# ruiqini/traj-opt-admm

Measured on AMD Instinct MI355X. Metric: ADMM iterations/sec, higher is better.
Workload: dtype f64

## Files before the change

### traj-opt-admm_amd/csrc/dev_common.h

```cpp
#pragma once
#include <hip/hip_runtime.h>
#include <stdint.h>
#include "dev_gjk.h"

namespace tj {

constexpr int WAVE = 64;
constexpr int STEP_CAP = 3332;
constexpr int NEWTON_CAP = 4000;
constexpr int MAX_LEVELS = 12;
constexpr int FRONT_CAP = 1024;

enum : int {
  ERR_PLANE_OVERFLOW = 1,
  ERR_FRONT_OVERFLOW = 2,
  ERR_LOOP_CAP = 4,
  ERR_PAIR_OVERFLOW = 8,
  ERR_NOT_SPD = 16,
  ERR_LS_RANGE = 32,
  ERR_CCD_STUCK = 128,
  ERR_SLACK_ARMIJO = 256,
  ERR_PLANE_REFINE = 64,
  ERR_PEER_TIMEOUT = 512,
  ERR_PASS_TIMEOUT = 1024,
// ... 85 lines not shown
  int rank[XCH_MAX];
  double* rx[XCH_MAX][2];
  unsigned long long* cnt[XCH_MAX];
};

struct Dev {
  int mode, U, P, res, S, T, N;
  int u0, u1;
  int rank, world;
  int xf;
  int c2_fold;
  int xf_all;
  __host__ __device__ int xf_want() const { return (xf_all || xs_async || fa_units) ? U : U - (u1 - u0); }
  __host__ __device__ int xf_units() const { return (xf && !xf_all) ? xf_want() * S : 0; }
  __host__ __device__ int xf_robot(int i) const { return xf_all ? i : (i < u0 ? i : i + (u1 - u0)); }
  int xch, xch_poll;
  const XchPeers* xp;
  int* xf_seg;
  double* rx[2];
  unsigned long long* xcnt;
  __host__ __device__ int n_foreign() const { return U - (u1 - u0); }
  __host__ __device__ int foreign_robot(int f) const { return f < u0 ? f : f + (u1 - u0); }
  __host__ __device__ int owner_of(int u) const { int r = (int)(((long long)(u + 1) * world - 1) / U); while ((long long)r * U / world > u) r--; while ((long long)(r + 1) * U / world <= u) r++; return r; }
  __host__ __device__ int owned_by(int r) const { return (int)((long long)(r + 1) * U / world) - (int)((long long)r * U / world); }
  int xs_async, xs_seq; int* xs_sync;
  __host__ __device__ int* xs_go() const { return xs_sync + ((size_t)2 * U + 1) * 32; }
  __host__ __device__ int* xs_ticket(int u) const { return xs_sync + (size_t)u * 32; }
  __host__ __device__ int* xs_flag(int u) const { return xs_sync + ((size_t)U + u) * 32; }
  __host__ __device__ int* xs_done() const { return xs_sync + (size_t)2 * U * 32; }
  __host__ __device__ static size_t xs_sync_ints(int U_) { return ((size_t)2 * U_ + 2) * 32; }
  int keep_async, keep_seq, keep_waves; int* keep_sync;
  __host__ __device__ int* keep_go() const { return keep_sync + 16 * 32; }
  __host__ __device__ static size_t keep_sync_ints() { return 17 * 32; }
  int fa, fa_units, fa_seq, fa_mid, fa_nls, fa_nfront; int* fa_sync;
  __host__ __device__ int* fa_res(int i) const { return fa_sync + (size_t)(i & 15) * 32; }
  __host__ __device__ int* fa_fdone(int i) const { return fa_sync + (size_t)(16 + (i & 15)) * 32; }
  __host__ __device__ int* fa_fstart(int i) const { return fa_sync + (size_t)(32 + (i & 15)) * 32; }
  __host__ __device__ int* fa_go(int i) const { return fa_sync + (size_t)(48 + (i & 63)) * 32; }
  __host__ __device__ int* fa_commit(int u) const { return fa_sync + (size_t)(112 + u) * 32; }
  __host__ __device__ int* fa_rec() const { return fa_sync + (size_t)(112 + U) * 32; }
  __host__ __device__ static size_t fa_sync_ints(int U_) { return (size_t)(113 + U_) * 32; }
  int lsc_follow;
  int xs_band;
  int seq_tree;
  int fuse;
  double lambda, margin, offset, mu, vel_limit, acc_limit, ks, kt, stop;
  int cap_obs, cap_self, cap_pairs;
  int optimal_plane;
  const double* basis;
  const double* convert;
  const double* mdyn;
  const double* kdop;
  const double* pow08;
  int prim;
  const double *px, *py, *pz;
  const double* tri;
  const float* leafbox;
  int nlevels;
  int bvh_skip;
  int lvl_off[MAX_LEVELS], lvl_n[MAX_LEVELS];
  const float* boxes;
  double *spline;
  double *p_slack;
  double *p_lambda;
  double *t_slack;
  double *t_lambda;
  double *piece_time;
  double *oplanes; int *ocount;
  double *splanes; int *scount;
  int *ocand, *ocand_n;
  double *ohull;
  int *obs_work, *obs_work_n;
  double *oraw; int *ostamp;
  double *hullinfo;
// ... 144 lines not shown
  sig_sent();
}
__device__ __forceinline__ void xf_wait_seg(const Dev& D, int kind, int tr) {
  const int want = D.xf_want();
  const int* w = xf_word(D, kind, tr);
  const long long lim = (D.xch || D.xs_async) ? WAIT_2S + WAIT_2S / 20 : WAIT_5MS + WAIT_SLACK * gridDim.x;
  if (!poll_until<2>([&] { return xf_load_i(w) >= want; }, lim)) wait_failed(D, ERR_LOOP_CAP | ERR_PASS_TIMEOUT);
}
template <int SLEEP = 2>
__device__ __forceinline__ void xs_wait(const Dev& D, const int* w, int want) {
  if (!poll_until<SLEEP>([&] { return xf_load_i(w) >= want; }, WAIT_2S)) wait_failed(D, ERR_LOOP_CAP | ERR_XS_TIMEOUT);
}
__device__ __forceinline__ int sum16(const int* base, int stride = 32) {
  int v = lane_id() < 16 ? xf_load_i(base + (size_t)lane_id() * stride) : 0;
  for (int o = 8; o > 0; o >>= 1) v += __shfl_xor(v, o);
  return __shfl(v, 0);
}
__device__ __forceinline__ void keep_wait(const Dev& D) {
  if (threadIdx.x < 64 && !poll_until<8>([&] { return sum16(D.keep_sync) >= D.keep_waves; }, WAIT_2S)) wait_failed(D, ERR_LOOP_CAP | ERR_XS_TIMEOUT);
  __syncthreads();
  asm volatile("" ::: "memory");
}
__device__ __forceinline__ void fa_wait16(const Dev& D, const int* base, int want) {
  if (!poll_until<4>([&] { return sum16(base) - want >= 0; }, WAIT_2S)) wait_failed(D, ERR_LOOP_CAP | ERR_XS_TIMEOUT);
}
__device__ __forceinline__ void fa_wait_flag(const Dev& D, const int* w, int want) {
  if (!poll_until<4>([&] { return xf_load_i(w) - want >= 0; }, WAIT_2S)) wait_failed(D, ERR_LOOP_CAP | ERR_XS_TIMEOUT);
}
__device__ __forceinline__ void fa_count(int* w) {
  sig_acked();
  if ((threadIdx.x & 63) == 0) __hip_atomic_fetch_add(w, 1, __ATOMIC_RELAXED, __HIP_MEMORY_SCOPE_AGENT);
  sig_sent();
}
__device__ __forceinline__ void xs_out(bool wt, double* p, double v) { if (wt) xf_store(p, v); else *p = v; }

constexpr int HULL_INFO_STRIDE = 128, HULL_BOX = 18, HULL_KLO = 24, HULL_KHI = 73;
__device__ __forceinline__ double* hull_record(const Dev& D, int u, int tr) { return D.hullinfo + ((size_t)u * D.S + tr) * HULL_INFO_STRIDE; }
__device__ __forceinline__ void hull_box_axis(const double* P, int a, double& lo, double& hi) {
  lo = INFINITY; hi = -INFINITY;
  for (int j = 0; j < 6; j++) { const double v = P[3 * j + a]; if (v < lo) lo = v; if (v > hi) hi = v; }
}
__device__ __forceinline__ void hull_kdop_axis(const Dev& D, const double* P, int ax, double& lo, double& up) {
  lo = INFINITY; up = -INFINITY;
  kdop_interval6(D.kdop[3 * ax], D.kdop[3 * ax + 1], D.kdop[3 * ax + 2], P, lo, up);
}
template <bool WT>
__device__ __forceinline__ void hull_record_put(const Dev& D, int u, int tr, int lane, double p, double blo, double bhi, double klo, double khi) {
  auto put = [](double* d, double v) { if constexpr (WT) xf_store(d, v); else *d = v; };
  double* o = hull_record(D, u, tr);
  if (lane < 18) put(o + lane, p);
  if (lane < 3) {
    put(o + HULL_BOX + lane, blo); put(o + HULL_BOX + 3 + lane, bhi);
    put(D.hbox + ((size_t)tr * 6 + lane) * D.U + u, blo); put(D.hbox + ((size_t)tr * 6 + 3 + lane) * D.U + u, bhi);
  }
  if (lane < 49) { put(o + HULL_KLO + lane, klo); put(o + HULL_KHI + lane, khi); }
}
template <bool WT>
__device__ __forceinline__ void hull_record_store(const Dev& D, int u, int tr, int lane, const double* P) {
  double blo = 0, bhi = 0, klo = 0, khi = 0;
  if (lane < 3) hull_box_axis(P, lane, blo, bhi);
  if (lane < 49) hull_kdop_axis(D, P, lane, klo, khi);
  hull_record_put<WT>(D, u, tr, lane, P[min(lane, 17)], blo, bhi, klo, khi);
}

__device__ __forceinline__ double* swept_record(const Dev& D, int u, int tr) { return D.ccdinfo + ((size_t)u * D.S + tr) * CCD_STRIDE; }
__device__ __forceinline__ BodySwept swept_body(const double* rec, double step) { return BodySwept{rec + CCD_P, rec + CCD_D, step}; }
// ... 81 lines not shown
```

### traj-opt-admm_amd/csrc/host_plan.h

```cpp
#pragma once
#include <algorithm>
#include <cstdlib>
#include <cstring>

namespace tj {

typedef const char* (*TuneFn)(const char* key);

struct KernelFact { int ok, regs, lds; };
struct PlanFacts {
  int num_cu;
  KernelFact xsolve;
  KernelFact grad[2];
  KernelFact front;
  int counters_on;
  int claim_refused;
  int prim, n_obs;
};
constexpr int PLAN_FACT_INTS = sizeof(PlanFacts) / sizeof(int);

struct HostPlan {
  size_t lds_grad = 0, lds_xs = 0, lds_xs2 = 0, lds_ls = 0, lds_seq = 0;
  LsLayout lsl;
  bool lsc_wide = false;
// ... 116 lines not shown
      auto gran = [](int r) { return (r + 7) / 8 * 8; };
      const int wx = XS_LOAD_THREADS / 64, wg = (h.grad_fold ? GRAD_FOLD_THREADS : GRAD_THREADS) / 64;
      const size_t lx = h.lds_xs + (size_t)ax.lds, lg = h.lds_grad_of(h.grad_fold, d.res) + (size_t)ag.lds;
      fits = ((wx + 3) / 4) * gran(ax.regs) + ((wg + 3) / 4) * gran(ag.regs) <= 512 && lx + lg <= (size_t)160 * 1024 && (wx + 3) / 4 + (wg + 3) / 4 <= 8;
    }
    if (!(2 * owned <= d.num_cu || (owned <= d.num_cu && fits))) d.xs_async = 0;
  }
  const char* const e_xs = tune("XS_ASYNC");
  const char* const e_keep = tune("KEEP_ASYNC");
  const bool xs_on = e_xs ? atoi(e_xs) != 0 : !f.counters_on, keep_on = e_keep ? atoi(e_keep) != 0 : !f.counters_on;
  d.xs_async = d.xs_async && xs_on;
  d.keep_async = (d.optimal_plane && decoupled && one && keep_on) ? 1 : 0;
  d.keep_waves = 1024;
  h.queues = 1 + d.xs_async + d.keep_async;
  h.forced = (e_xs && atoi(e_xs) != 0) || (e_keep && atoi(e_keep) != 0);
  if (f.claim_refused) { d.xs_async = 0; d.keep_async = 0; h.hwq_refused = true; }
  h.xs_two_queues = d.xs_async && tune("XS_ONE_QUEUE") == nullptr;
  h.keep_two_queues = d.keep_async != 0;
  if (const char* e = tune("GRAD_BALANCE")) d.grad_bal = (atoi(e) != 0 && owned * d.P <= 65536) ? 1 : 0;
  if (const char* e = tune("LS_HELP")) { h.ls_help_forced = true; h.ls_help_asked = atoi(e); }
  d.ls_help = plan_ls_help(d, h, d.num_cu);
  if (const char* e = tune("LS_HELP_LATE")) d.ls_help_late = std::max(0, std::min(4000, atoi(e)));
  d.ls_help_mute = flag(tune("LS_HELP_MUTE"), 0);
  d.fa = (d.xs_async && one && !d.optimal_plane &&
          (!coupled ? (d.fuse && owned * d.ls_help <= d.num_cu) : (h.lsc_wide && d.xf_all && owned * LSC_ROUNDS <= d.num_cu))) ? flag(tune("FRONT_ASYNC"), 1) : 0;
  h.fa_emulate = flag(tune("FRONT_ASYNC_ONE_QUEUE"), 0) != 0;
  if (d.fa) {
    h.fa_mid_front = plan_grids(d, h.n_solve_env).n_front;
    if (f.front.ok) {
      const int by_lds = (int)(((size_t)160 * 1024) / std::max<size_t>((size_t)f.front.lds, 1)), by_regs = 4 * (512 / std::max((f.front.regs + 7) / 8 * 8, 8)), per_cu = std::min(std::min(by_lds, by_regs), 32);
      h.fa_mid_ok = (long long)h.fa_mid_front <= (long long)(d.num_cu - 1) * per_cu;
    }
    h.fa_mid_ok = h.fa_mid_ok && flag(tune("FRONT_ASYNC_MID"), 1);
  }
  h.heal = flag(tune("HEAL"), 1) != 0;
  if (const char* e = tune("XS_FAULT")) h.xs_fault = atoi(e);
  if (h.lds_grad_of(true, d.res) > lds_max || h.lds_xs > lds_max || h.lds_ls > lds_max || h.lds_seq > lds_max)
    return fail("problem does not fit the 160 KB LDS of one CU (segments per robot / fleet size too large for this version)");
  return pl;
}

#ifdef TJ_KAT
inline int plan_record(const Plan& pl, const PlanFacts& f, int* out, int cap) {
  const Dev& d = pl.d; const HostPlan& h = pl.h;
  const Grids g = plan_grids(d, h.n_solve_env);
  const int v[] = {
    pl.err, d.mode, d.U, d.P, d.res, d.S, d.T, d.N, d.prim, d.u0, d.u1, d.rank, d.world, d.fuse, d.xf, d.xf_all, d.cap_obs, d.cap_self, d.cap_pairs, d.optimal_plane,
    d.pair_rows, d.cap_work, d.xs, d.grad_npl, d.xs_band, d.seq_tree, d.bvh_skip, d.pair_prio, d.mid_order, d.pair_lpw, d.pair_pass_on, d.spec, d.seq_fold, d.spec_budget,
    d.spec_min, d.ls_fast, d.num_cu, d.c2_fold, d.grad_bal, d.xs_async, d.keep_async, d.keep_waves, d.ls_help, d.ls_help_late, d.ls_help_mute, d.fa,
    h.grad_fold, h.n_solve_env, h.lsc_wide, h.fa_emulate, h.fa_mid_ok, h.fa_mid_front, h.hwq_refused, h.queues, h.forced, h.xs_two_queues, h.keep_two_queues, h.heal, h.xs_fault,
    (int)h.lds_grad, (int)h.lds_xs, (int)h.lds_xs2, (int)h.lds_ls, (int)h.lds_seq, (int)h.lsl.total, h.lsl.plane_cap, h.lsl.affine, h.lsl.groups,
    g.n_rows, g.n_ccd, g.n_xf, g.n_front, g.n_solve, g.n_obs_solve, g.n_mid_slack};
  const int nv = (int)(sizeof(v) / sizeof(int)), n = PLAN_FACT_INTS + nv;
  if (cap < n) return -n;
  memcpy(out, &f, sizeof(f)); memcpy(out + PLAN_FACT_INTS, v, sizeof(v));
  return n;
}
#endif

}
```

### traj-opt-admm_amd/csrc/kernels_pairs.h

```cpp
#pragma once
#include "dev_common.h"
#include "dev_linalg.h"
#include "kernels_sep.h"

namespace tj {

__global__ __launch_bounds__(64) void k_hullinfo(Dev D) {
  if (TJ_DONE(D)) return;
  const int u = blockIdx.x / D.S, tr = blockIdx.x % D.S, lane = lane_id();
  __shared__ double P[18];
  if (lane < 18) P[lane] = hull_entry(D, D.spline + (size_t)u * 3 * D.T, tr, lane / 3, lane % 3);
  __syncthreads();
  hull_record_store<false>(D, u, tr, lane, P);
}

__host__ __device__ inline int pair_units(int U, int R) {
  const int nc = (U + 63) / 64;
  int n = 0;
  for (int g = 0; 64 * g < U - 1; g++) { const int rows = min(64 * g + 64, U - 1) - 64 * g; n += ((rows + R - 1) / R) * (nc - g); }
  return n;
}
__host__ __device__ inline void pair_unit(int U, int R, int bid, int& tr, int& rb, int& cb) {
  const int per = pair_units(U, R), nc = (U + 63) / 64;
  tr = bid / per;
// ... 386 lines not shown
}
template <bool FA>
__device__ __forceinline__ void pair_dedicated(const Dev& D, int b, unsigned key, bool have_early, const PairSolve& early, bool head_start, int spec_thr, int epoch, int lane,
                                               double* A, double* B, const int* wpre) {
  auto ldi = [&](const int* p) { if constexpr (FA) return xf_load_i(p); else return *p; };
  __builtin_amdgcn_s_setprio(3);
  TJ_TIC(D, K_SEP_SELF_SOLVE, 0);
  const PairId id = pair_unkey(key);
  if (!pair_id_valid(D, id)) return;
  GjkState hs; bool hs_fin = false;
  if (!have_early) {
    pair_hull_put(A, B, lane, pair_hull_fetch<FA>(D, id, lane));
    spec_state_load<FA>(D, b, lane, hs, hs_fin);
  }
  const int cnt = wpre[id.tr + 1] - wpre[id.tr];
  const int* wl = D.pair_work + 3 * (size_t)id.tr * pair_work_cap_seg(D);
  bool member = false;
  for (int i = lane; i < cnt; i += 64) member = member || (ldi(wl + 3 * i + 1) == id.p0 && ldi(wl + 3 * i + 2) == id.q);
  __syncthreads();
  TJ_TIC(D, K_SEP_SELF_SOLVE, 1);
  PairSolve r = early;
  if (!have_early) r = pair_solve_wave(D, A, B, lane, hs, true, hs_fin);
#ifdef TJ_PHASE_TIMING
  if (lane == 0 && blockIdx.x < TJ_TIC_BLOCKS) { D.dbg[((size_t)K_SEP_SELF_SOLVE * TJ_TIC_BLOCKS + blockIdx.x) * TJ_TIC_SLOTS + 6] = r.gjk + 1000; D.dbg[((size_t)K_SEP_SELF_SOLVE * TJ_TIC_BLOCKS + blockIdx.x) * TJ_TIC_SLOTS + 7] = r.ok ? r.newton : -1; }
#endif
  if (ballot(member)) {
    if (lane == 0) atomicAdd(&D.ctl->spec_taken, 1);
    pair_note_slow(D, id, r.gjk, epoch, lane, head_start, spec_thr);
    pair_result_store(D, id, r, epoch, lane);
  }
  TJ_TIC(D, K_SEP_SELF_SOLVE, 2);
}
template <bool FA>
__device__ __forceinline__ void pair_generic(const Dev& D, int r, int Wg, int n, const SpecTags& tags, bool head_start, int spec_thr, int epoch, int lane,
                                             double* A, double* B, const int* wpre) {
  auto ldi = [&](const int* p) { if constexpr (FA) return xf_load_i(p); else return *p; };
  if (r >= n) return;
  TJ_TIC(D, K_SEP_SELF_SOLVE, 0);
  int it_tr = 0, it_p0 = 0, it_q = 0;
  const int n_mine = (n - r + Wg - 1) / Wg;
  if (n_mine > 64) { if (lane == 0) atomicOr(&D.ctl->error, ERR_PAIR_OVERFLOW); return; }
  if (lane < n_mine) {
    const size_t sl = (size_t)pair_work_slot(D, wpre, r + lane * Wg);
    it_tr = ldi(D.pair_work + 3 * sl); it_p0 = ldi(D.pair_work + 3 * sl + 1); it_q = ldi(D.pair_work + 3 * sl + 2);
  }
  auto item = [&](int j) { return PairId{__builtin_amdgcn_readlane(it_tr, j), __builtin_amdgcn_readlane(it_p0, j), __builtin_amdgcn_readlane(it_q, j)}; };
  PairId next = item(0);
  double hv = pair_hull_fetch<FA>(D, next, lane);
  for (int j = 0; j < n_mine; j++) {
    const bool first = j == 0;
    __syncthreads();
    pair_hull_put(A, B, lane, hv);
    __syncthreads();
    const PairId id = next;
    if (j + 1 < n_mine) {
      next = item(j + 1);
      hv = pair_hull_fetch<FA>(D, next, lane);
    }
    if (first) TJ_TIC(D, K_SEP_SELF_SOLVE, 1);
    if (head_start && tags.holds(pair_tag_word(epoch, pair_key(id)))) continue;
    GjkState gs;
    const PairSolve s = pair_solve_wave(D, A, B, lane, gs, false, false,
#ifdef TJ_PHASE_LIGHT
                                        nullptr);
#else
                                        first ? &D : nullptr);
#endif
#ifdef TJ_PHASE_TIMING
    if (lane == 0 && first && blockIdx.x < TJ_TIC_BLOCKS) { D.dbg[((size_t)K_SEP_SELF_SOLVE * TJ_TIC_BLOCKS + blockIdx.x) * TJ_TIC_SLOTS + 6] = s.gjk; D.dbg[((size_t)K_SEP_SELF_SOLVE * TJ_TIC_BLOCKS + blockIdx.x) * TJ_TIC_SLOTS + 7] = s.ok ? s.newton : -1; }
#endif
    pair_note_slow(D, id, s.gjk, epoch, lane, head_start, spec_thr);
    pair_result_store(D, id, s, epoch, lane);
    if (first) TJ_TIC(D, K_SEP_SELF_SOLVE, 2);
  }
}

template <bool FA = false>
__device__ __forceinline__ void sep_self_solve_body(const Dev& D, int bid, int nwaves, bool head_start, double* tile) {
  const int lane = lane_id();
  __shared__ double A[18], B[18];
  __shared__ int wpre[513];
  auto ldt = [&](const unsigned long long* p) { if constexpr (FA) return __hip_atomic_load(p, __ATOMIC_RELAXED, __HIP_MEMORY_SCOPE_AGENT); else return *p; };
  const int n_ded = min(nwaves / 2, SPEC_CAP);
  bool have_early = false; PairSolve early{false, false, 0, 0, 0, 0, 0, 0};
  if constexpr (FA) {
    if (head_start && bid < n_ded) have_early = pair_early_head_start(D, bid, lane, A, B, early);
    fa_wait_flag(D, D.fa_go(bid), D.fa_seq);
  }
  const unsigned long long spec_tag0 = head_start ? ldt(D.spec_tag + lane) : 0ull, spec_tag1 = head_start ? ldt(D.spec_tag + 64 + lane) : 0ull;
  const int spec_thr = head_start ? max(D.spec_min, D.ctl->gjk_prev - SPEC_GJK_WINDOW) : 0;
  const int n = pair_work_prefix<FA>(D, wpre, lane);
  const int epoch = D.ctl->epoch;
  if (n > 4 * nwaves) {
    const PairLanePlan pl = pair_lane_plan(D, n, nwaves);
    if (pl.pass_on && bid >= pl.np) pair_consumer<FA>(D, bid - pl.np, pl, nwaves, epoch, lane, A, B);
    else pair_lane_producer<FA>(D, bid, nwaves, n, pl, epoch, lane, wpre, tile);
    return;
  }
  const SpecTags tags = spec_tags(spec_tag0, spec_tag1, head_start, epoch, n_ded, lane);
  if (tags.dedicated(bid)) pair_dedicated<FA>(D, bid, tags.key_of(bid), have_early, early, head_start, spec_thr, epoch, lane, A, B, wpre);
  else pair_generic<FA>(D, bid - tags.below(bid), nwaves - tags.count(), n, tags, head_start, spec_thr, epoch, lane, A, B, wpre);
}
__global__ __launch_bounds__(64) void k_sep_self_solve(Dev D) {
  if (TJ_DONE(D)) return;
  __shared__ double tile[PAIR_TILE_DOUBLES];
  sep_self_solve_body(D, blockIdx.x, gridDim.x, false, tile);
}

__device__ __forceinline__ void compact_segment(const Dev& D, int u, int tr, int lane, double* pst_o = nullptr, double* pst_s = nullptr, int* cnt = nullptr, int pst_cap = 0, int* fits = nullptr) {
  const int U = D.U, epoch = D.ctl->epoch;
  const size_t seg = (size_t)u * D.S + tr;
  const bool obs_part = !(D.optimal_plane && !D.multi());
  const bool pair_part = D.multi();
  const int n = obs_part ? D.ocand_n[seg] : 0;
  const int W = (U + 63) >> 6;
  unsigned long long* bw = D.pairbits + ((size_t)tr * U + u) * W;
  unsigned long long wbits = 0;
  if (pair_part && lane < W) wbits = bw[lane];
  double* outp = D.splanes + seg * D.cap_self * 4;
  int pbase = 0;
  if (pair_part) {
    for (int q0 = 0; q0 < U; q0 += 64) {
      const unsigned long long word = __shfl(wbits, q0 >> 6);
      if (word == 0ull) continue;
      const int q = q0 + lane;
      const bool bit = (word >> lane) & 1ull;
      const size_t slot = ((size_t)tr * U + u) * U + min(q, U - 1);
      int st = 0; double v0 = 0, v1 = 0, v2 = 0, v3 = 0;
      if (bit && q < U) { st = D.pairstamp[slot]; const double* p = D.pairplane + 4 * slot; v0 = p[0]; v1 = p[1]; v2 = p[2]; v3 = p[3]; }
      const bool ok = bit && q < U && q != u && st == epoch;
      const unsigned long long mask = ballot(ok);
      const int idx = pbase + prefix_count(mask);
      if (ok) {
        if (idx < D.cap_self) {
// ... 44 lines not shown
```

### traj-opt-admm_amd/csrc/kernels_step.h

```cpp
#pragma once
#include "dev_common.h"
#include "dev_linalg.h"
#include "kernels_sep.h"
#include "kernels_ls.h"
#include "kernels_pairs.h"
#include "dev_dyntree.h"

namespace tj {

template <bool XF = false>
__device__ __forceinline__ void ccd_prep_segment(const Dev& D, const double* net, const double* dir, int u, int tr, int lane, double* sh, int sysdir = 0) {
  double* P = sh; double* Dh = sh + 18; double* PD = sh + 36; double* PS = sh + 54;
  auto ldd = [&](const double* p) { return (XF && sysdir == 1) ? xch_load(p) : ((XF && sysdir == 2) ? xf_load(p) : *p); };
  auto st = [&](double* p, double v) { if constexpr (XF) xf_store(p, v); else *p = v; };
  const int e = lane % 18, r0 = div_small(tr, D.res) * 3 + D.T * (e % 3);
  const double* B = D.basis + (size_t)tr * 36 + (e / 3) * 6;
  if (lane < 18) P[lane] = hull_sum(B, net + r0);
  else if (lane < 54) {
    double dk[6];
#pragma unroll
    for (int k = 0; k < 6; k++) dk[k] = ldd(dir + r0 + k);
    if (lane < 36) Dh[e] = hull_sum(B, dk); else PD[e] = hull_sum_pd(B, net + r0, dk);
  }
  blk_sync<true>();
// ... 549 lines not shown
  __host__ __device__ __forceinline__ int total() const { return obs + pt.count(); }
  __host__ __device__ __forceinline__ explicit FrontLayout(const Dev& d) : pt(d) {
    ord = d.grad_bal ? ((d.u1 - d.u0) * d.P + 63) / 64 : 0;
    xf = ord + d.xf_units();
    spec = xf + (d.spec ? SPEC_CAP : 0);
    obs = spec + owned_segments(d);
  }
};
struct MidLayout {
  enum Body { SLACK, PAIR, OBS };
  __host__ __device__ __forceinline__ static int slack_blocks(const Dev& d) { return (d.u1 - d.u0) * d.P; }
  int watcher, slack0, n_slack, pair0, n_pair, obs0, n_obs, total;
  __host__ __device__ __forceinline__ MidLayout(const Dev& d, int n_pair_waves, int n_obs_waves, bool with_watcher, bool slack_last) {
    watcher = with_watcher ? 1 : 0; n_slack = slack_blocks(d); n_pair = n_pair_waves; n_obs = n_obs_waves;
    pair0 = slack_last ? 0 : n_slack; obs0 = pair0 + n_pair; slack0 = slack_last ? obs0 + n_obs : 0;
    total = watcher + n_slack + n_pair + n_obs;
  }
  __host__ __device__ __forceinline__ Body body(int b) const { return (unsigned)(b - slack0) < (unsigned)n_slack ? SLACK : ((unsigned)(b - pair0) < (unsigned)n_pair ? PAIR : OBS); }
};
struct CcdLayout {
  int fin, xf, obs; PairTiles pt;
  __host__ __device__ __forceinline__ explicit CcdLayout(const Dev& d) : pt(d) {
    fin = d.seq_fold ? 1 : 0;
    xf = fin + d.xf_units();
    obs = xf + owned_segments(d);
  }
  __host__ __device__ __forceinline__ int tiles() const { return pt.count(); }
  __host__ __device__ __forceinline__ int total() const { return obs + tiles(); }
};
template <int PRIM, bool FA = false>
__global__ __launch_bounds__(64) void k_front(Dev D) {
  if (D.keep_seq > 0 && blockIdx.x == 0 && threadIdx.x == 0) __hip_atomic_store(D.keep_go(), D.keep_seq, __ATOMIC_RELAXED, __HIP_MEMORY_SCOPE_AGENT);
  int fa_epoch = 0;
  if constexpr (FA) {
    if (threadIdx.x == 0) __hip_atomic_fetch_add(D.fa_fstart(blockIdx.x), 1, __ATOMIC_RELAXED, __HIP_MEMORY_SCOPE_AGENT);
    fa_epoch = xf_load_i(D.fa_rec() + 1);
    if (xf_load_i(D.fa_rec() + 2) | (D.ctl->error & ERR_XS_TIMEOUT)) { fa_count(D.fa_fdone(blockIdx.x)); return; }
  } else if (TJ_DONE(D)) return;
  TJ_TIC(D, K_FRONT, 0);
  __shared__ double lds[OBS_LDS_DOUBLES > PAIR_LDS_DOUBLES ? OBS_LDS_DOUBLES : PAIR_LDS_DOUBLES];
  static_assert(sizeof(lds) >= GRAD_ORDER_CHUNK * sizeof(int), "grad_order_body stages its costs in this buffer");
  const FrontLayout L(D);
  const int bx = (int)blockIdx.x;
  const bool pub = D.xf_all != 0 || (D.fa_units != 0 && D.multi());
  if (bx < L.ord) grad_order_body<FA>(D, bx, (int*)lds);
  else if (bx < L.xf) xf_hull_body(D, bx - L.ord);
  else if (bx < L.spec) spec_pair_body<FA>(D, bx - L.xf, lds, fa_epoch);
  else if (bx < L.obs) obs_query_body<PRIM, FA>(D, bx - L.spec, lds, !pub, pub);
  else sep_self_rows_body<FA>(D, bx - L.obs, lds, D.xf != 0 || D.fa_units != 0);
  TJ_TIC(D, K_FRONT, 1);
  if constexpr (FA) fa_count(D.fa_fdone(blockIdx.x));
}
__global__ __launch_bounds__(64) void k_fa_gate(Dev D, int want) { fa_wait16(D, D.fa_res(0), want); }
template <int PRIM, bool FA, bool SLACK_LAST>
__device__ __forceinline__ void mid_dispatch(const Dev& D, int b, int n_pair_waves, int n_obs_waves, double* mid_lds) {
  const MidLayout L(D, n_pair_waves, n_obs_waves, FA, SLACK_LAST);
  const MidLayout::Body body = L.body(b);
  if (body == MidLayout::SLACK) { if (D.ctl->slack_now) slack_body(D, b - L.slack0, 1, mid_lds); TJ_TIC(D, K_MID, 1); return; }
  if (TJ_DONE(D)) return;
  if (body == MidLayout::PAIR) sep_self_solve_body<FA>(D, b - L.pair0, n_pair_waves, D.spec != 0, mid_lds);
  else { if constexpr (FA) { fa_wait_flag(D, D.fa_go(b), D.fa_seq); if constexpr (!SLACK_LAST) TJ_TIC(D, K_MID, 4); } obs_solve_body<PRIM, FA>(D, b - L.obs0, n_obs_waves); }
  TJ_TIC(D, K_MID, 1);
}
template <int PRIM, bool FA = false>
__global__ __launch_bounds__(64) __attribute__((amdgpu_waves_per_eu(2, 2))) void k_mid(Dev D, int n_pair_waves, int n_obs_waves) {
  constexpr int watcher = FA ? 1 : 0;
  if constexpr (FA) {
    if ((int)blockIdx.x < watcher) {
      fa_wait16(D, D.fa_fdone(0), (int)((unsigned)D.fa_seq * (unsigned)D.fa_nfront));
      sig_acked();
      xf_store_i(D.fa_go(threadIdx.x), D.fa_seq);
      sig_sent();
      return;
    }
  }
  const int b = (int)blockIdx.x - watcher;
  TJ_TIC(D, K_MID, 0);
#ifdef TJ_PHASE_TIMING
  if (threadIdx.x == 0 && blockIdx.x < TJ_TIC_BLOCKS) {
    D.dbg[((size_t)K_MID * TJ_TIC_BLOCKS + blockIdx.x) * TJ_TIC_SLOTS + 2] = __builtin_amdgcn_s_getreg((31 << 11) | 4);
    D.dbg[((size_t)K_MID * TJ_TIC_BLOCKS + blockIdx.x) * TJ_TIC_SLOTS + 3] = __builtin_amdgcn_s_getreg((31 << 11) | 20);
  }
#endif
  __shared__ double mid_lds[SLACK_LDS_DOUBLES > PAIR_TILE_DOUBLES ? SLACK_LDS_DOUBLES : PAIR_TILE_DOUBLES];
// ... 92 lines not shown
```

### traj-opt-admm_amd/csrc/tj_api.hip

```cpp
#include <hip/hip_runtime.h>
#include <cstdio>
#include <cstdlib>
#include <cstring>
#include <strings.h>
#include <string>
#include <type_traits>
#include <vector>
#include "../../include/trajadmm.h"
#include "dev_common.h"
#include "host_tables.h"
#include "kernels_sep.h"
#include "kernels_pairs.h"
#include "kernels_keep.h"
#include "kernels_newton.h"
#include "kernels_step.h"
#ifdef TJ_KAT
#include "../../include/trajadmm_kat.h"
#include "kernels_debug.h"
#endif
#include "kernels_plan.h"
#include "kernels_bvh.h"
#include "kernels_audit.h"
#include "kernels_audit_timed.h"
#include "kernels_closest.h"
// ... 202 lines not shown
  return TJ_OK;
}


int ensure_hull_cache(tj_ctx* c);

int flush_deferred(tj_ctx* c) {
  if (!c->maybe_deferred) return TJ_OK;
  const Dev& d = c->d;
  TJ_LAUNCH(k_flush, dim3(1), dim3(1), 0, c->stream, d, c->begin_folded ? 1 : 0);
  c->begin_folded = false;
  TJ_LAUNCH(k_slack, dim3((d.u1 - d.u0) * d.P), dim3(64), 0, c->stream, d, 1);
  HIPCHK(c, hipGetLastError());
  c->maybe_deferred = false;
  return TJ_OK;
}

#define QUIESCE_NOHEAL(c)                                       \
  do {                                                          \
    int qr_ = flush_deferred(c);                                \
    if (qr_) return qr_;                                        \
    HIPCHK(c, hipStreamSynchronize((c)->stream));               \
    if ((c)->xq.stream2) HIPCHK(c, hipStreamSynchronize((c)->xq.stream2)); \
    if ((c)->xq.stream3) HIPCHK(c, hipStreamSynchronize((c)->xq.stream3)); \
  } while (0)
#define QUIESCE(c)                                              \
  do {                                                          \
    QUIESCE_NOHEAL(c);                                          \
    if ((c)->snap_iters > 0 && !(c)->heal_busy) { int hr_ = heal_check(c, -1); if (hr_) return hr_; } \
  } while (0)

int restart_pairings(tj_ctx* c, bool keep_go) {
  HIPCHK(c, hipMemsetAsync(c->d.xs_sync, 0, (keep_go ? (size_t)(c->d.xs_go() - c->d.xs_sync) : Dev::xs_sync_ints(c->d.U)) * sizeof(int), c->stream));
  HIPCHK(c, hipMemsetAsync(c->d.fa_sync, 0, Dev::fa_sync_ints(c->d.U) * sizeof(int), c->stream)); c->ss.fa_seq = 0; c->ss.fa_armed = c->ss.fa_mid_now = false;
  if (!keep_go) { HIPCHK(c, hipMemsetAsync(c->d.keep_sync, 0, Dev::keep_sync_ints() * sizeof(int), c->stream)); c->ss.xs_seq = c->ss.xs_seq_gated = c->ss.keep_seq = 0; }
  return TJ_OK;
}
int checkpoint_take(tj_ctx* c, bool in_begin) {
  Checkpoint& k = c->ck;
  c->ss.ck_in_begin = in_begin; k.begin_folded = c->begin_folded; k.maybe_deferred = c->maybe_deferred; k.lsc_base = c->ss.lsc_base;
  if (!in_begin) { hipLaunchKernelGGL(k_snapshot, dim3(64, std::max(k.n, 1)), dim3(256), 0, c->stream, k.tab, k.n, 0, c->d.ctl, k.ctl); HIPCHK(c, hipGetLastError()); }
  return TJ_OK;
}
int checkpoint_restore(tj_ctx* c) {
  const Checkpoint& k = c->ck;
  hipLaunchKernelGGL(k_snapshot, dim3(64, std::max(k.n, 1)), dim3(256), 0, c->stream, k.tab, k.n, 1, c->d.ctl, k.ctl); HIPCHK(c, hipGetLastError());
  c->begin_folded = k.begin_folded; c->maybe_deferred = k.maybe_deferred; c->ss.lsc_base = k.lsc_base; c->hull_valid = c->ss.ccd_valid = c->ss.xf_used[0] = c->ss.xf_used[1] = false;
  return c->begin_folded ? flush_deferred(c) : TJ_OK;
}
void checkpoint_drop(tj_ctx* c) { c->ss.ck_in_begin = 0; }

int heal_check(tj_ctx* c, int err_known) {
  int err = err_known;
  if (err < 0) HIPCHK(c, hipMemcpy(&err, &c->d.ctl->error, sizeof(int), hipMemcpyDeviceToHost));
  const long long n = c->snap_iters; c->snap_iters = 0;
  if (!(err & ERR_XS_TIMEOUT)) { checkpoint_drop(c); return TJ_OK; }
  struct Busy { tj_ctx* c; ~Busy() { c->heal_busy = false; } } busy{c}; c->heal_busy = true;
  c->async_fallbacks++;
  release_queues(c);
  c->ss.xs_two_queues = c->ss.keep_two_queues = false; c->ss.xs_fault = 0;
  int r = restart_pairings(c, false);
  if (r || (r = checkpoint_restore(c))) return r;
  checkpoint_drop(c);
  HIPCHK(c, hipMemsetAsync(c->d.xf_seg, 0, (size_t)2 * c->d.S * XF_SEG_STRIDE * sizeof(int), c->stream)); HIPCHK(c, hipMemsetAsync(c->d.spec_n, 0, 8, c->stream));
  if ((r = tj_iterate_async(c, (int)n))) return r;
  QUIESCE_NOHEAL(c);
  return TJ_OK;
// ... 157 lines not shown
    if (!r) r = upload(c, q, src, n * sizeof(*q));
    dst = q;
    return r;
  };
  int r;
  if ((r = put(d.basis, t.basis.data(), t.basis.size())) || (r = put(d.convert, t.convert.data(), t.convert.size())) || (r = put(d.mdyn, t.mdyn, 36)) ||
      (r = put(d.kdop, t.kdop, 147)) || (r = put(d.pow08, t.pow08.data(), t.pow08.size())) || (r = put(d.xs_gather, gt.data(), gt.size()))) return r;
  return TJ_OK;
}

struct ArrayDecl { void** slot; size_t n, elem; bool snap; };
template <class T>
ArrayDecl arr(T*& p, size_t n, bool snap = false) { return ArrayDecl{(void**)&p, n, sizeof(T), snap}; }
constexpr bool SNAP = true;

std::vector<ArrayDecl> device_arrays(Dev& d) {
  const size_t U = d.U, S = d.S, P = d.P, T = d.T, owned = d.u1 - d.u0, n = 9 * P - 2, co = d.cap_obs, cs = d.cap_self;
  const bool multi = d.mode >= 1;
  std::vector<ArrayDecl> a = {
    arr(d.spline, U * 3 * T, SNAP), arr(d.p_slack, U * 18 * P, SNAP), arr(d.p_lambda, U * 18 * P, SNAP), arr(d.t_slack, U * P, SNAP), arr(d.t_lambda, U * P, SNAP), arr(d.piece_time, U, SNAP),
    arr(d.oplanes, U * S * co * 4), arr(d.ocount, U * S), arr(d.splanes, U * S * cs * 4), arr(d.scount, U * S),
    arr(d.lg, U * P * 19), arr(d.lh, U * P * 361), arr(d.xdir, U * d.xs, SNAP),
    arr(d.k_obs, U), arr(d.k_self, U), arr(d.step_out, U, SNAP), arr(d.ls_hist, U, SNAP), arr(d.grad_cost, owned * P), arr(d.grad_perm, owned * P), arr(d.ls_tab, U * LS_TAB_STRIDE), arr(d.ls_word, U),
    arr(d.ccdinfo, U * S * CCD_STRIDE), arr(d.pair_list, ACT_CAP),
    arr(d.seg_stats, U * S * 6, SNAP), arr(d.pair_stats, U * S * 2, SNAP), arr(d.blk_stats, U * P + U, SNAP),
    arr(d.hullinfo, U * S * HULL_INFO_STRIDE), arr(d.hbox, S * 6 * U), arr(d.cbox, S * 6 * U), arr(d.pairplane, multi ? S * U * U * 4 : 1),
    arr(d.pairstamp, multi ? S * U * U : 1), arr(d.pairbits, multi ? S * U * ((U + 63) / 64) : 1),
    arr(d.pair_work, 3 * (size_t)d.cap_work), arr(d.pair_work_n, S + 1), arr(d.pair_ovf, 4), arr(d.seq_gmem_d, SeqLayout(d.U, ACT_CAP, true).tree_doubles), arr(d.seq_gmem_i, SeqLayout(d.U, ACT_CAP, true).tree_ints),
    arr(d.spec_n, 2), arr(d.spec_list, 2 * SPEC_CAP), arr(d.spec_tag, SPEC_CAP), arr(d.spec_state, SPEC_CAP * SPEC_STATE_DOUBLES), arr(d.spec_sti, SPEC_CAP * SPEC_STATE_INTS),
    arr(d.pair_ovf_list, (size_t)d.cap_work + PAIR_CONSUMERS_MAX), arr(d.ctl, 1),
    arr(d.ocand, U * S * co), arr(d.ocand_n, U * S), arr(d.ohull, U * S * 18),
    arr(d.obs_work, 2 * U * S * co), arr(d.obs_work_n, 1), arr(d.oraw, U * S * co * 4), arr(d.ostamp, U * S * co),
    arr(d.grad_scr, owned * P * 16 * (co + cs)), arr(d.xs_scr, d.xs_band ? owned * (n * n + 4 * n) : 1),
    arr(d.xf_seg, 2 * S * XF_SEG_STRIDE), arr(d.xs_sync, Dev::xs_sync_ints(d.U)), arr(d.keep_sync, Dev::keep_sync_ints()), arr(d.fa_sync, Dev::fa_sync_ints(d.U))};
#ifdef TJ_PHASE_TIMING
  a.push_back(arr(d.dbg, (size_t)K_COUNT * TJ_TIC_BLOCKS * TJ_TIC_SLOTS));
#endif
  if (d.optimal_plane) {
    const bool m0 = d.mode == 0;
    a.insert(a.end(), {arr(d.kobs_id, m0 ? U * S * co : 1, m0), arr(d.kobs_n, U * S, m0), arr(d.kobs_cd, m0 ? U * S * co * 4 : 1, m0),
                       arr(d.kpair_on, m0 ? 1 : S * U * U, !m0), arr(d.kpair_list, m0 ? 1 : S * U * U, !m0), arr(d.kpair_n, 2, !m0), arr(d.kpair_cd, m0 ? 1 : S * U * U * 4, !m0)});
  }
  if (d.mode == TJ_MODE_MULTI_COUPLED)
    a.insert(a.end(), {arr(d.xL, U * (d.xs_band ? (n - 1) * BAND_BS + n : n * n)), arr(d.xy, U * n), arr(d.xg, U * n), arr(d.xcorner, U * 4), arr(d.k_obs_f, U), arr(d.ls_e, (size_t)LSC_ROUNDS * U * LS_GROUPS)});
  return a;
}

int allocate_arrays(tj_ctx* c) {
  const std::vector<ArrayDecl> arrays = device_arrays(c->d);
  int r;
  for (const ArrayDecl& a : arrays) if ((r = dalloc_bytes(c, a.slot, std::max<size_t>(a.n, 1) * a.elem))) return r;
  std::vector<SnapRegion> tab;
  for (const ArrayDecl& a : arrays) {
    if (!a.snap) continue;
    char* snap = nullptr;
    if ((r = dalloc(c, &snap, (a.n * a.elem + 15) / 16 * 16))) return r;
    tab.push_back(SnapRegion{(char*)*a.slot, snap, (unsigned long long)(a.n * a.elem)});
  }
  c->ck.n = (int)tab.size();
  if ((r = dalloc(c, &c->ck.tab, tab.size())) || (r = dalloc(c, &c->ck.ctl, 1)) || (r = upload(c, c->ck.tab, tab.data(), tab.size() * sizeof(SnapRegion)))) return r;
  return TJ_OK;
}

}

extern "C" {

// ... 1628 lines not shown
```

Baseline: 6185.

## Release pair-solve waves per segment as front tiles finish

```diff
diff --git a/traj-opt-admm_amd/csrc/dev_common.h b/traj-opt-admm_amd/csrc/dev_common.h
--- a/traj-opt-admm_amd/csrc/dev_common.h
+++ b/traj-opt-admm_amd/csrc/dev_common.h
@@ -141,14 +141,17 @@
   int keep_async, keep_seq, keep_waves; int* keep_sync;
   __host__ __device__ int* keep_go() const { return keep_sync + 16 * 32; }
   __host__ __device__ static size_t keep_sync_ints() { return 17 * 32; }
-  int fa, fa_units, fa_seq, fa_mid, fa_nls, fa_nfront; int* fa_sync;
+  int fa, fa_units, fa_seq, fa_mid, fa_nls, fa_nfront, pair_seg, fa_ntile; int* fa_sync;
   __host__ __device__ int* fa_res(int i) const { return fa_sync + (size_t)(i & 15) * 32; }
   __host__ __device__ int* fa_fdone(int i) const { return fa_sync + (size_t)(16 + (i & 15)) * 32; }
   __host__ __device__ int* fa_fstart(int i) const { return fa_sync + (size_t)(32 + (i & 15)) * 32; }
   __host__ __device__ int* fa_go(int i) const { return fa_sync + (size_t)(48 + (i & 63)) * 32; }
   __host__ __device__ int* fa_commit(int u) const { return fa_sync + (size_t)(112 + u) * 32; }
   __host__ __device__ int* fa_rec() const { return fa_sync + (size_t)(112 + U) * 32; }
-  __host__ __device__ static size_t fa_sync_ints(int U_) { return (size_t)(113 + U_) * 32; }
+  __host__ __device__ int* fa_seg(int tr) const { return fa_sync + (size_t)(113 + U + tr) * 32; }
+  __host__ __device__ int* fa_hs() const { return fa_sync + (size_t)(113 + U + S) * 32; }
+  __host__ __device__ int* fa_listed(int par) const { return fa_sync + (size_t)(114 + U + S) * 32 + (size_t)par * (((size_t)S + 32) & ~(size_t)31); }
+  __host__ __device__ static size_t fa_sync_ints(int U_, int S_) { return (size_t)(114 + U_ + S_) * 32 + 2 * (((size_t)S_ + 32) & ~(size_t)31); }
   int lsc_follow;
   int xs_band;
   int seq_tree;
@@ -359,6 +362,14 @@
   if ((threadIdx.x & 63) == 0) __hip_atomic_fetch_add(w, 1, __ATOMIC_RELAXED, __HIP_MEMORY_SCOPE_AGENT);
   sig_sent();
 }
+__device__ __forceinline__ void fa_count2(int* group, int* w) {
+  sig_acked();
+  if ((threadIdx.x & 63) == 0) {
+    if (group) __hip_atomic_fetch_add(group, 1, __ATOMIC_RELAXED, __HIP_MEMORY_SCOPE_AGENT);
+    __hip_atomic_fetch_add(w, 1, __ATOMIC_RELAXED, __HIP_MEMORY_SCOPE_AGENT);
+  }
+  sig_sent();
+}
 __device__ __forceinline__ void xs_out(bool wt, double* p, double v) { if (wt) xf_store(p, v); else *p = v; }
 
 constexpr int HULL_INFO_STRIDE = 128, HULL_BOX = 18, HULL_KLO = 24, HULL_KHI = 73;
diff --git a/traj-opt-admm_amd/csrc/host_plan.h b/traj-opt-admm_amd/csrc/host_plan.h
--- a/traj-opt-admm_amd/csrc/host_plan.h
+++ b/traj-opt-admm_amd/csrc/host_plan.h
@@ -172,6 +172,8 @@
       h.fa_mid_ok = (long long)h.fa_mid_front <= (long long)(d.num_cu - 1) * per_cu;
     }
     h.fa_mid_ok = h.fa_mid_ok && flag(tune("FRONT_ASYNC_MID"), 1);
+    d.fa_ntile = d.mode >= 1 ? pair_units(d.U, d.pair_rows) : 0;
+    d.pair_seg = (h.fa_mid_ok && d.mode >= 1 && d.fa_ntile > 0) ? flag(tune("PAIR_SEG_RELEASE"), 1) : 0;
   }
   h.heal = flag(tune("HEAL"), 1) != 0;
   if (const char* e = tune("XS_FAULT")) h.xs_fault = atoi(e);
diff --git a/traj-opt-admm_amd/csrc/kernels_pairs.h b/traj-opt-admm_amd/csrc/kernels_pairs.h
--- a/traj-opt-admm_amd/csrc/kernels_pairs.h
+++ b/traj-opt-admm_amd/csrc/kernels_pairs.h
@@ -442,32 +442,25 @@
   TJ_TIC(D, K_SEP_SELF_SOLVE, 2);
 }
 template <bool FA>
-__device__ __forceinline__ void pair_generic(const Dev& D, int r, int Wg, int n, const SpecTags& tags, bool head_start, int spec_thr, int epoch, int lane,
-                                             double* A, double* B, const int* wpre) {
-  auto ldi = [&](const int* p) { if constexpr (FA) return xf_load_i(p); else return *p; };
-  if (r >= n) return;
-  TJ_TIC(D, K_SEP_SELF_SOLVE, 0);
-  int it_tr = 0, it_p0 = 0, it_q = 0;
-  const int n_mine = (n - r + Wg - 1) / Wg;
-  if (n_mine > 64) { if (lane == 0) atomicOr(&D.ctl->error, ERR_PAIR_OVERFLOW); return; }
-  if (lane < n_mine) {
-    const size_t sl = (size_t)pair_work_slot(D, wpre, r + lane * Wg);
-    it_tr = ldi(D.pair_work + 3 * sl); it_p0 = ldi(D.pair_work + 3 * sl + 1); it_q = ldi(D.pair_work + 3 * sl + 2);
-  }
+__device__ __forceinline__ void pair_solve_items(const Dev& D, int n_mine, int it_tr, int it_p0, int it_q, const SpecTags& tags, bool head_start, int spec_thr, int epoch, int lane,
+                                                 double* A, double* B, bool stamps) {
+  if (n_mine <= 0) return;
   auto item = [&](int j) { return PairId{__builtin_amdgcn_readlane(it_tr, j), __builtin_amdgcn_readlane(it_p0, j), __builtin_amdgcn_readlane(it_q, j)}; };
+  auto listed = [&](const PairId& id) { return (unsigned)id.tr < (unsigned)D.S && (unsigned)id.p0 < (unsigned)D.U && (unsigned)id.q < (unsigned)D.U; };
   PairId next = item(0);
-  double hv = pair_hull_fetch<FA>(D, next, lane);
+  double hv = listed(next) ? pair_hull_fetch<FA>(D, next, lane) : 0.0;
   for (int j = 0; j < n_mine; j++) {
-    const bool first = j == 0;
+    const bool first = stamps && j == 0;
     __syncthreads();
     pair_hull_put(A, B, lane, hv);
     __syncthreads();
     const PairId id = next;
     if (j + 1 < n_mine) {
       next = item(j + 1);
-      hv = pair_hull_fetch<FA>(D, next, lane);
+      hv = listed(next) ? pair_hull_fetch<FA>(D, next, lane) : 0.0;
     }
     if (first) TJ_TIC(D, K_SEP_SELF_SOLVE, 1);
+    if (!listed(id)) continue;
     if (head_start && tags.holds(pair_tag_word(epoch, pair_key(id)))) continue;
     GjkState gs;
     const PairSolve s = pair_solve_wave(D, A, B, lane, gs, false, false,
@@ -484,6 +477,94 @@
     if (first) TJ_TIC(D, K_SEP_SELF_SOLVE, 2);
   }
 }
+__device__ __forceinline__ int pair_prefix_row(const int* pre, int S, int x) {
+  int lo = 0, hi = S;
+  while (hi - lo > 1) { const int mid = (lo + hi) >> 1; if (pre[mid] <= x) lo = mid; else hi = mid; }
+  return lo;
+}
+template <class F>
+__device__ __forceinline__ void pair_prefix_of(int S, int* pre, int lane, F&& f) {
+  int run = 0;
+  for (int base = 0; base < S; base += 64) {
+    const int tr = base + lane;
+    const int c = tr < S ? f(tr) : 0;
+    int x = c;
+#pragma unroll
+    for (int off = 1; off < 64; off <<= 1) { const int y = __shfl_up(x, off); if (lane >= off) x += y; }
+    if (tr < S) pre[tr] = run + x - c;
+    run += __shfl(x, 63);
+  }
+  if (lane == 0) pre[S] = run;
+  __builtin_amdgcn_fence(__ATOMIC_ACQ_REL, "workgroup"); __builtin_amdgcn_wave_barrier();
+}
+
+constexpr int PAIR_SEG_ITEMS = 8;
+__device__ __forceinline__ void pair_seg_bind(int S, int* bind, const int* prev, bool known, int Wg, int lane) {
+  unsigned C = 0; int nz = 0;
+  for (int base = 0; base < S; base += 64) { const unsigned c = (known && base + lane < S) ? (unsigned)prev[base + lane] : 0u; C += c; nz += c ? 1 : 0; }
+  for (int o = 32; o > 0; o >>= 1) { C += __shfl_xor(C, o); nz += __shfl_xor(nz, o); }
+  const bool prop = C > 0u && nz <= Wg;
+  const unsigned spare = prop ? (unsigned)(Wg - nz) : 0u;
+  pair_prefix_of(S, bind, lane, [&](int tr) {
+    if (!prop) return Wg / S + (tr < Wg % S ? 1 : 0);
+    const unsigned c = (unsigned)prev[tr];
+    return c ? min(1 + (int)(c * spare / C), (int)c) : 0;
+  });
+}
+template <bool FA>
+__device__ __forceinline__ bool pair_seg_pass(const Dev& D, int r, int Wg, const SpecTags& tags, bool head_start, int spec_thr, int epoch, int lane, double* A, double* B,
+                                              int* bind, const int* prev, bool known) {
+  const int S = D.S, cap = pair_work_cap_seg(D);
+  pair_seg_bind(S, bind, prev, known, Wg, lane);
+  if (r >= bind[S]) return true;
+  const int tr = __builtin_amdgcn_readfirstlane(pair_prefix_row(bind, S, r));
+  const int k = r - __builtin_amdgcn_readfirstlane(bind[tr]), w = max(__builtin_amdgcn_readfirstlane(bind[tr + 1] - bind[tr]), 1);
+  fa_wait_flag(D, D.fa_seg(tr), (int)((unsigned)D.fa_seq * (unsigned)D.fa_ntile));
+  TJ_TIC(D, K_SEP_SELF_SOLVE, 0);
+#ifdef TJ_PHASE_TIMING
+  if (lane == 0 && blockIdx.x < TJ_TIC_BLOCKS) D.dbg[((size_t)K_MID * TJ_TIC_BLOCKS + blockIdx.x) * TJ_TIC_SLOTS + 5] = tr + 1;
+#endif
+  int it_tr = -1, it_p0 = 0, it_q = 0;
+  const int idx = k + lane * w;
+  if (lane < PAIR_SEG_ITEMS && idx < cap) {
+    const size_t sl = (size_t)tr * cap + idx;
+    it_tr = xf_load_i(D.pair_work + 3 * sl); it_p0 = xf_load_i(D.pair_work + 3 * sl + 1); it_q = xf_load_i(D.pair_work + 3 * sl + 2);
+  }
+  const int cnt = __builtin_amdgcn_readfirstlane(min(xf_load_i(D.pair_work_n + tr), cap));
+  const int n_mine = cnt > k ? min(PAIR_SEG_ITEMS, (cnt - k + w - 1) / w) : 0;
+  pair_solve_items<FA>(D, n_mine, it_tr, it_p0, it_q, tags, head_start, spec_thr, epoch, lane, A, B, true);
+  return k == w - 1;
+}
+template <bool FA>
+__device__ __forceinline__ void pair_generic(const Dev& D, int r, int Wg, const SpecTags& tags, bool head_start, int spec_thr, int epoch, int lane,
+                                             double* A, double* B, const int* wpre, const int* bind = nullptr, int* spre = nullptr, int* tpre = nullptr) {
+  auto ldi = [&](const int* p) { if constexpr (FA) return xf_load_i(p); else return *p; };
+  const int S = D.S, cap = pair_work_cap_seg(D);
+  auto covered = [&](int tr) { return bind ? min(wpre[tr + 1] - wpre[tr], PAIR_SEG_ITEMS * (bind[tr + 1] - bind[tr])) : 0; };
+  const int* pre = wpre;
+  if (bind) {
+    pair_prefix_of(S, spre, lane, [&](int tr) { return wpre[tr + 1] - wpre[tr] - covered(tr); }); pre = spre;
+    if (pre[S] == 0) return;
+    pair_prefix_of(S, tpre, lane, [&](int tr) { return bind[tr + 1] > bind[tr] ? 1 : 0; });
+    const int nb = tpre[S];
+    r = r >= bind[S] ? nb + (r - bind[S]) : tpre[pair_prefix_row(bind, S, r)];
+    Wg = nb + (Wg - bind[S]);
+  }
+  const int n = pre[S];
+  if (r >= n) return;
+  if (!bind) TJ_TIC(D, K_SEP_SELF_SOLVE, 0);
+  const int n_all = (n - r + Wg - 1) / Wg;
+  for (int j0 = 0; j0 < n_all; j0 += 64) {
+    int it_tr = -1, it_p0 = 0, it_q = 0;
+    const int n_mine = min(n_all - j0, 64);
+    if (lane < n_mine) {
+      const int x = r + (j0 + lane) * Wg, tr = pair_prefix_row(pre, S, x);
+      const size_t sl = (size_t)tr * cap + covered(tr) + (x - pre[tr]);
+      it_tr = ldi(D.pair_work + 3 * sl); it_p0 = ldi(D.pair_work + 3 * sl + 1); it_q = ldi(D.pair_work + 3 * sl + 2);
+    }
+    pair_solve_items<FA>(D, n_mine, it_tr, it_p0, it_q, tags, head_start, spec_thr, epoch, lane, A, B, !bind && j0 == 0);
+  }
+}
 
 template <bool FA = false>
 __device__ __forceinline__ void sep_self_solve_body(const Dev& D, int bid, int nwaves, bool head_start, double* tile) {
@@ -493,15 +574,39 @@
   auto ldt = [&](const unsigned long long* p) { if constexpr (FA) return __hip_atomic_load(p, __ATOMIC_RELAXED, __HIP_MEMORY_SCOPE_AGENT); else return *p; };
   const int n_ded = min(nwaves / 2, SPEC_CAP);
   bool have_early = false; PairSolve early{false, false, 0, 0, 0, 0, 0, 0};
+  bool seg = false;
   if constexpr (FA) {
     if (head_start && bid < n_ded) have_early = pair_early_head_start(D, bid, lane, A, B, early);
-    fa_wait_flag(D, D.fa_go(bid), D.fa_seq);
-  }
-  const unsigned long long spec_tag0 = head_start ? ldt(D.spec_tag + lane) : 0ull, spec_tag1 = head_start ? ldt(D.spec_tag + 64 + lane) : 0ull;
+    seg = D.pair_seg && nwaves <= 65535;
+    if (!seg || have_early) fa_wait_flag(D, D.fa_go(bid), D.fa_seq);
+  }
+  unsigned long long spec_tag0 = head_start ? ldt(D.spec_tag + lane) : 0ull, spec_tag1 = head_start ? ldt(D.spec_tag + 64 + lane) : 0ull;
   const int spec_thr = head_start ? max(D.spec_min, D.ctl->gjk_prev - SPEC_GJK_WINDOW) : 0;
+  const int epoch = D.ctl->epoch;
+  int* const bind = (int*)tile; int* const spre = bind + 520; int* const tpre = bind + 1040;
+  static_assert(PAIR_TILE_DOUBLES * sizeof(double) >= 3 * 520 * sizeof(int), "the tile holds the three tables");
+  if constexpr (FA) {
+    if (seg && !have_early) {
+      const int* listed = D.fa_listed((epoch & 1) ^ 1);
+      const int listed_epoch = xf_load_i(listed);
+      for (int tr = lane; tr < D.S; tr += 64) spre[tr] = min(max(xf_load_i(listed + 1 + tr), 0), 65535);
+      __builtin_amdgcn_fence(__ATOMIC_ACQ_REL, "workgroup"); __builtin_amdgcn_wave_barrier();
+      if (head_start && ballot((int)(spec_tag0 >> 32) != epoch || (int)(spec_tag1 >> 32) != epoch) != 0ull) {
+        fa_wait_flag(D, D.fa_hs(), (int)((unsigned)D.fa_seq * (unsigned)SPEC_CAP));
+        spec_tag0 = ldt(D.spec_tag + lane); spec_tag1 = ldt(D.spec_tag + 64 + lane);
+      }
+      const SpecTags tags = spec_tags(spec_tag0, spec_tag1, head_start, epoch, n_ded, lane);
+      if (!tags.dedicated(bid) && !pair_seg_pass<FA>(D, bid - tags.below(bid), nwaves - tags.count(), tags, head_start, spec_thr, epoch, lane, A, B, bind, spre, listed_epoch == epoch - 1)) return;
+      fa_wait_flag(D, D.fa_go(bid), D.fa_seq);
+    }
+  }
   const int n = pair_work_prefix<FA>(D, wpre, lane);
-  const int epoch = D.ctl->epoch;
-  if (n > 4 * nwaves) {
+  if (D.pair_seg && bid == nwaves - 1) {
+    int* out = D.fa_listed(epoch & 1);
+    for (int tr = lane; tr < D.S; tr += 64) xf_store_i(out + 1 + tr, wpre[tr + 1] - wpre[tr]);
+    if (lane == 0) xf_store_i(out, epoch);
+  }
+  if (!seg && n > 4 * nwaves) {
     const PairLanePlan pl = pair_lane_plan(D, n, nwaves);
     if (pl.pass_on && bid >= pl.np) pair_consumer<FA>(D, bid - pl.np, pl, nwaves, epoch, lane, A, B);
     else pair_lane_producer<FA>(D, bid, nwaves, n, pl, epoch, lane, wpre, tile);
@@ -509,7 +614,7 @@
   }
   const SpecTags tags = spec_tags(spec_tag0, spec_tag1, head_start, epoch, n_ded, lane);
   if (tags.dedicated(bid)) pair_dedicated<FA>(D, bid, tags.key_of(bid), have_early, early, head_start, spec_thr, epoch, lane, A, B, wpre);
-  else pair_generic<FA>(D, bid - tags.below(bid), nwaves - tags.count(), n, tags, head_start, spec_thr, epoch, lane, A, B, wpre);
+  else pair_generic<FA>(D, bid - tags.below(bid), nwaves - tags.count(), tags, head_start, spec_thr, epoch, lane, A, B, wpre, seg ? bind : nullptr, spre, tpre);
 }
 __global__ __launch_bounds__(64) void k_sep_self_solve(Dev D) {
   if (TJ_DONE(D)) return;
diff --git a/traj-opt-admm_amd/csrc/kernels_step.h b/traj-opt-admm_amd/csrc/kernels_step.h
--- a/traj-opt-admm_amd/csrc/kernels_step.h
+++ b/traj-opt-admm_amd/csrc/kernels_step.h
@@ -605,16 +605,18 @@
 __global__ __launch_bounds__(64) void k_front(Dev D) {
   if (D.keep_seq > 0 && blockIdx.x == 0 && threadIdx.x == 0) __hip_atomic_store(D.keep_go(), D.keep_seq, __ATOMIC_RELAXED, __HIP_MEMORY_SCOPE_AGENT);
   int fa_epoch = 0;
+  const FrontLayout L(D);
+  const int bx = (int)blockIdx.x;
+  int* fa_group = nullptr;
   if constexpr (FA) {
     if (threadIdx.x == 0) __hip_atomic_fetch_add(D.fa_fstart(blockIdx.x), 1, __ATOMIC_RELAXED, __HIP_MEMORY_SCOPE_AGENT);
+    if (D.pair_seg) fa_group = bx >= L.obs ? D.fa_seg((bx - L.obs) / D.fa_ntile) : ((bx >= L.xf && bx < L.spec) ? D.fa_hs() : nullptr);
     fa_epoch = xf_load_i(D.fa_rec() + 1);
-    if (xf_load_i(D.fa_rec() + 2) | (D.ctl->error & ERR_XS_TIMEOUT)) { fa_count(D.fa_fdone(blockIdx.x)); return; }
+    if (xf_load_i(D.fa_rec() + 2) | (D.ctl->error & ERR_XS_TIMEOUT)) { fa_count2(fa_group, D.fa_fdone(blockIdx.x)); return; }
   } else if (TJ_DONE(D)) return;
   TJ_TIC(D, K_FRONT, 0);
   __shared__ double lds[OBS_LDS_DOUBLES > PAIR_LDS_DOUBLES ? OBS_LDS_DOUBLES : PAIR_LDS_DOUBLES];
   static_assert(sizeof(lds) >= GRAD_ORDER_CHUNK * sizeof(int), "grad_order_body stages its costs in this buffer");
-  const FrontLayout L(D);
-  const int bx = (int)blockIdx.x;
   const bool pub = D.xf_all != 0 || (D.fa_units != 0 && D.multi());
   if (bx < L.ord) grad_order_body<FA>(D, bx, (int*)lds);
   else if (bx < L.xf) xf_hull_body(D, bx - L.ord);
@@ -622,7 +624,7 @@
   else if (bx < L.obs) obs_query_body<PRIM, FA>(D, bx - L.spec, lds, !pub, pub);
   else sep_self_rows_body<FA>(D, bx - L.obs, lds, D.xf != 0 || D.fa_units != 0);
   TJ_TIC(D, K_FRONT, 1);
-  if constexpr (FA) fa_count(D.fa_fdone(blockIdx.x));
+  if constexpr (FA) fa_count2(fa_group, D.fa_fdone(blockIdx.x));
 }
 __global__ __launch_bounds__(64) void k_fa_gate(Dev D, int want) { fa_wait16(D, D.fa_res(0), want); }
 template <int PRIM, bool FA, bool SLACK_LAST>
diff --git a/traj-opt-admm_amd/csrc/tj_api.hip b/traj-opt-admm_amd/csrc/tj_api.hip
--- a/traj-opt-admm_amd/csrc/tj_api.hip
+++ b/traj-opt-admm_amd/csrc/tj_api.hip
@@ -258,7 +258,7 @@
 
 int restart_pairings(tj_ctx* c, bool keep_go) {
   HIPCHK(c, hipMemsetAsync(c->d.xs_sync, 0, (keep_go ? (size_t)(c->d.xs_go() - c->d.xs_sync) : Dev::xs_sync_ints(c->d.U)) * sizeof(int), c->stream));
-  HIPCHK(c, hipMemsetAsync(c->d.fa_sync, 0, Dev::fa_sync_ints(c->d.U) * sizeof(int), c->stream)); c->ss.fa_seq = 0; c->ss.fa_armed = c->ss.fa_mid_now = false;
+  HIPCHK(c, hipMemsetAsync(c->d.fa_sync, 0, Dev::fa_sync_ints(c->d.U, c->d.S) * sizeof(int), c->stream)); c->ss.fa_seq = 0; c->ss.fa_armed = c->ss.fa_mid_now = false;
   if (!keep_go) { HIPCHK(c, hipMemsetAsync(c->d.keep_sync, 0, Dev::keep_sync_ints() * sizeof(int), c->stream)); c->ss.xs_seq = c->ss.xs_seq_gated = c->ss.keep_seq = 0; }
   return TJ_OK;
 }
@@ -482,7 +482,7 @@
     arr(d.ocand, U * S * co), arr(d.ocand_n, U * S), arr(d.ohull, U * S * 18),
     arr(d.obs_work, 2 * U * S * co), arr(d.obs_work_n, 1), arr(d.oraw, U * S * co * 4), arr(d.ostamp, U * S * co),
     arr(d.grad_scr, owned * P * 16 * (co + cs)), arr(d.xs_scr, d.xs_band ? owned * (n * n + 4 * n) : 1),
-    arr(d.xf_seg, 2 * S * XF_SEG_STRIDE), arr(d.xs_sync, Dev::xs_sync_ints(d.U)), arr(d.keep_sync, Dev::keep_sync_ints()), arr(d.fa_sync, Dev::fa_sync_ints(d.U))};
+    arr(d.xf_seg, 2 * S * XF_SEG_STRIDE), arr(d.xs_sync, Dev::xs_sync_ints(d.U)), arr(d.keep_sync, Dev::keep_sync_ints()), arr(d.fa_sync, Dev::fa_sync_ints(d.U, d.S))};
 #ifdef TJ_PHASE_TIMING
   a.push_back(arr(d.dbg, (size_t)K_COUNT * TJ_TIC_BLOCKS * TJ_TIC_SLOTS));
 #endif
```

Result: slower. 6085 (-1.6%).
